# Metronlab/bow

Measured on AMD Instinct MI355X. Metric: rows/sec rolling-mean on 1B-row float64, higher is better.
Workload: dtype f64; 1 GPU; IntervalRolling(interval=10, offset=0)+Aggregate(WindowStart,ArithmeticMean), dense int64 ts=i + float64 u01 values, 1000000000 rows/GPU resident in HBM, null_count=0; rows_per_gpu=1000000000, windows_per_gpu=100000000, parallelism=rows range-partitioned x1

## Files before the change

### bow_amd/capi.py

```python
import contextlib
import ctypes as C
import os

import numpy as np

_HERE = os.path.dirname(os.path.abspath(__file__))
LIB_PATH = os.environ.get("BOWGPU_LIB") or os.path.join(_HERE, "libbowgpu.so")

FLOAT64, INT64, BOOLEAN, STRING = 1, 2, 3, 4
HOST, DEVICE, HOST_PINNED = 0, 1, 2
TYPE_NAMES = {"float64": FLOAT64, "int64": INT64, "bool": BOOLEAN, "utf8": STRING}

AGG = {
    "WindowStart": 0, "Sum": 1, "ArithmeticMean": 2, "Min": 3, "Max": 4, "Count": 5, "First": 6,
    "Last": 7, "IntegralStep": 8, "IntegralTrapezoid": 9, "WeightedAverageStep": 10,
    "WeightedAverageLinear": 11, "NumRows": 12, "Mode": 13,
}
INTERP = {"WindowStart": 0, "Linear": 1, "StepPrevious": 2, "None": 3, "Const": 4}

MAX_FACTORS = 4
BOOL_LANE_ROWS = 256
FILTER_MAX_VALUES = 32
FILTER_MAX_PREDS = 8
CARRY_MAX_AGGS = 16
# ... 148 lines not shown
    return _lib


def page_aligned(count, dtype, fill=None):
    nbytes = max(count, 1) * np.dtype(dtype).itemsize
    raw = np.empty(((nbytes + 4095) // 4096 + 1) * 4096, dtype=np.uint8)
    off = (-raw.ctypes.data) % 4096
    arr = raw[off:off + nbytes].view(dtype)
    if fill is not None:
        arr[:] = fill
    return arr


def host_register(arr):
    check(lib().bowgpu_host_register(arr.ctypes.data_as(C.c_void_p), C.c_int64(arr.nbytes)))


def host_unregister(arr):
    check(lib().bowgpu_host_unregister(arr.ctypes.data_as(C.c_void_p)))


def set_devices(ids, min_rows=None):
    ids = list(ids)
    arr = (C.c_int * max(len(ids), 1))(*ids)
    check(lib().bowgpu_set_devices(arr, len(ids)))
    if min_rows is not None:
        check(lib().bowgpu_set_fanout_min_rows(C.c_int64(min_rows)))


def get_devices():
    n = C.c_int(0)
    arr = (C.c_int * 64)()
    check(lib().bowgpu_get_devices(arr, 64, C.byref(n)))
    return [arr[i] for i in range(n.value)]


def fanout_counts():
    a, b = C.c_int64(0), C.c_int64(0)
    check(lib().bowgpu_fanout_counts(C.byref(a), C.byref(b)))
    return a.value, b.value


def last_call_ranks():
    n = C.c_int(0)
    check(lib().bowgpu_last_call_ranks(C.byref(n)))
    return n.value


class devices:

    def __init__(self, ids, min_rows=None):
        self.ids, self.min_rows = list(ids), min_rows

    def __enter__(self):
        self.prev = get_devices()
        set_devices(self.ids, self.min_rows)
        return self

    def __exit__(self, *exc):
        set_devices(self.prev, (1 << 20) if self.min_rows is not None else None)
        return False


def mem_info():
    f, t = C.c_int64(0), C.c_int64(0)
    check(lib().bowgpu_mem_info(C.byref(f), C.byref(t)))
    return f.value, t.value


def trim(all_threads=True):
    n = C.c_int64(0)
    check(lib().bowgpu_trim(1 if all_threads else 0, C.byref(n)))
    return n.value


def check(rc):
    if rc != 0:
        raise BowGpuError(rc, lib().bowgpu_last_error().decode("utf-8", "replace"))


ROUTE_NO_SIMPLE, ROUTE_FORCE_GENERAL, ROUTE_NO_LONG_ONLY, ROUTE_LONG_CLASSIC, ROUTE_LONG_STREAM_ALL = 1, 2, 4, 8, 16
ROUTE_SIMPLE_SMALL_LIST, ROUTE_SIMPLE_LARGE_LIST, ROUTE_TW_F64, ROUTE_SIMPLE_PADDED, ROUTE_INTERP_TILE = 32, 64, 128, 256, 512
ROUTE_PINNED_STAGE, ROUTE_STRICT_ORDER, ROUTE_NO_FUSED, ROUTE_TW_ROWS, ROUTE_INTERP_COPIES = 1024, 2048, 4096, 8192, 16384
ROUTE_QUEUE_HOST, ROUTE_QUEUE_DEVICE = 32768, 65536


def set_route(mask):
    check(lib().bowgpu_debug_set_route(C.c_uint32(mask)))


def get_route():
    m = C.c_uint32(0)
    check(lib().bowgpu_debug_get_route(C.byref(m)))
    return m.value


class route:

    def __init__(self, mask):
        self.mask = mask

    def __enter__(self):
        self.prev = get_route()
        set_route(self.mask)
        return self

    def __exit__(self, *exc):
        set_route(self.prev)
        return False


AGG_ROUTES = (("auto", 0), ("classic-long", ROUTE_LONG_CLASSIC), ("stream-all", ROUTE_LONG_STREAM_ALL),
              ("small-list", ROUTE_SIMPLE_SMALL_LIST), ("large-list", ROUTE_SIMPLE_LARGE_LIST), ("padded", ROUTE_SIMPLE_PADDED), ("tw-rows", ROUTE_TW_ROWS),
              ("queue-device", ROUTE_NO_LONG_ONLY | ROUTE_QUEUE_DEVICE), ("queue-host", ROUTE_NO_LONG_ONLY | ROUTE_QUEUE_HOST),
              ("lean", ROUTE_NO_SIMPLE | ROUTE_NO_LONG_ONLY), ("general", ROUTE_FORCE_GENERAL | ROUTE_NO_LONG_ONLY))
INTERP_ROUTES = (("wave3", 0), ("tile", ROUTE_INTERP_TILE))


def agg_routes():
    for label, mask in AGG_ROUTES:
        with route(mask):
            yield label


class DeviceBuffer:

    def __init__(self, nbytes):
        self.nbytes = int(nbytes)
        p = C.c_void_p()
        check(lib().bowgpu_malloc(C.byref(p), C.c_int64(self.nbytes)))
        self.ptr = p.value

    @classmethod
    def from_numpy(cls, arr):
        arr = np.ascontiguousarray(arr)
        b = cls(max(arr.nbytes, 8))
        if arr.nbytes:
            check(lib().bowgpu_memcpy_h2d(C.c_void_p(b.ptr), arr.ctypes.data_as(C.c_void_p), C.c_int64(arr.nbytes)))
        return b

    def to_numpy(self, dtype, count, first=0):
        out = np.empty(count, dtype=dtype)
        if out.nbytes:
            check(lib().bowgpu_memcpy_d2h(out.ctypes.data_as(C.c_void_p), C.c_void_p(self.ptr + first * out.itemsize), C.c_int64(out.nbytes)))
        return out

    def free(self):
        if self.ptr:
            lib().bowgpu_free(C.c_void_p(self.ptr))
            self.ptr = None

    def __del__(self):
        try:
            self.free()
        except Exception:
            pass


class Column:

    def __init__(self, values, validity=None, typ=None, offset=0, length=None, null_count=-1):
        if isinstance(values, DeviceBuffer):
            self.residency = DEVICE
            assert typ is not None and length is not None
            self.values, self.validity = values, validity
        else:
            self.residency = HOST
# ... 900 lines not shown
```

### bow_amd/csrc/agg_pass.cpp

```cpp

#include <stdio.h>
#include <stdlib.h>
#include <string.h>
#include <time.h>

#include "agg_host.h"

namespace bowgpu {

static int64_t compact_long_max_rows(uint32_t need) {
    if ((need & kNeedTimeWeighted) == kNeedTimeWeighted || (need & kNeedMinMax)) return kCompactLongBothMaxAvgRows;
    if (need & (kNeedTimeWeighted | kNeedFirstLast)) return kCompactLongMaxAvgRows;
    return 0;
}
static bool ids_and_times_fit(const Plan &plan, int64_t slot0, int64_t W) {
    const int64_t lim53 = 1ll << 53;
    return plan.first_ts > -lim53 && plan.last_ts < lim53 && (uint64_t)plan.last_ts - (uint64_t)slot0 < 0xFFFFFFF0ull && W < 0xFFFFFFF0ll;
}

int job_build(Ctx *c, const AggCall &call, const bowgpu_agg *aggs, int32_t naggs, bowgpu_out *outs, int64_t wid_base, int64_t W,
              bool holds_row0, AggJob *job, int nullable_per_pass) {
    pending_drop(c);
    const bowgpu_col *cols = call.cols;
    const int32_t ncols = call.ncols, ts_col = call.ts_col;
// ... 129 lines not shown
        const bowgpu_out *u = job->douts[i].user;
        b->user[i] = (u && u->residency == BOWGPU_DEVICE) ? u->validity : nullptr;
        b->ones[i] = all_ones || kind_never_nil(job->aggs[i].kind);
        b->count[i] = !kind_never_nil(job->aggs[i].kind);
    }
    if (preset && job->check_plan) { b->check_ts = job->P.ts; b->check_n = job->P.n; b->check_first = job->plan.first_ts; b->check_last = job->plan.last_ts; }
}

static int job_enqueue_tail(Ctx *c, AggJob *job) {
    const int64_t W = job->W;
    if (W > 0) {
        BitmapBatch b;
        job_bitmaps(job, false, false, &b);
        if (W <= kFinishHostBits) {
            BG_TRY(ctx_pinned(c, 16384, reinterpret_cast<void **>(&b.host_block)));
            job->tail_wrote_host = true;
        } else if (job->counts_used) BG_HIP(hipMemsetAsync(b.counts, 0, 8 * kMaxAggs, c->stream));
        BG_TRY(launch_finish_bitmaps(c, b));
        job->counts_used = true;
    }
    for (int i = 0; i < job->naggs; i++) BG_TRY(devout_finish(c, &job->douts[i], W, job->P.aggs[i].out_type, 0, false));
    return 0;
}

static int job_readback(Ctx *c, AggJob *job, uint32_t **hstat, uint64_t **hcnt) {
    char *hp;
    BG_TRY(ctx_pinned(c, 16384, reinterpret_cast<void **>(&hp)));
    if (job->tail_wrote_host) job->tail_wrote_host = false;
    else BG_HIP(hipMemcpyAsync(hp, job->P.status, kReadbackBytes, hipMemcpyDeviceToHost, c->stream));
    *hstat = reinterpret_cast<uint32_t *>(hp);
    *hcnt = reinterpret_cast<uint64_t *>(hp + kCountsOffset);
    return 0;
}

static int job_settle_enqueue(Ctx *c, AggJob *job, bool tail, uint32_t **hstat, uint64_t **hcnt) {
    if (tail) BG_TRY(job_enqueue_tail(c, job));
    return job_readback(c, job, hstat, hcnt);
}
static int job_settle(Ctx *c, AggJob *job, bool tail, uint32_t **hstat, uint64_t **hcnt) {
    BG_TRY(job_settle_enqueue(c, job, tail, hstat, hcnt));
    BG_HIP(hipStreamSynchronize(c->stream));
    return 0;
}

int fail_ts_unsorted() { return fail(BOWGPU_ERR_TS_UNSORTED, "interval column is not ascending: outside the device path"); }

constexpr uint32_t kLookPlan = 1u << kAggStPlanMismatch, kLookUnsorted = 1u << kAggStUnsorted, kLookOverflow = 1u << kAggStListOverflow,
                   kLookStrict = 1u << kAggStStrictTooLong;
static int agg_status_error(const uint32_t *hstat, uint32_t look) {
    if ((look & kLookPlan) && hstat[kAggStPlanMismatch])
        return fail(BOWGPU_ERR_ARG, "the plan was not made for this interval column (its first / last timestamp differ)");
    if ((look & kLookUnsorted) && hstat[kAggStUnsorted]) return fail_ts_unsorted();
    if ((look & kLookOverflow) && hstat[kAggStListOverflow]) return fail(BOWGPU_ERR_HIP, "internal: long-window list overflow");
    if ((look & kLookStrict) && hstat[kAggStStrictTooLong])
        return fail(BOWGPU_ERR_UNSUPPORTED, "strict_order: some window holds more than 2^20 rows (one lane walks a window in row order: beyond that the call is declined)");
    return 0;
}

static void job_null_counts(AggJob *job, const uint64_t *hcnt) {
    for (int i = 0; i < job->naggs; i++)
        job->douts[i].user->null_count = (job->W > 0 && !kind_never_nil(job->aggs[i].kind)) ? job->W - (int64_t)hcnt[i] : 0;
}

static bool simple_applies(const AggJob *job, bool time_weighted, bool *is_int, bool *has_nulls, bool *wide) {
    const AggParams &P = job->P;
    const Plan &plan = job->plan;
    if ((job->inclusive && !time_weighted) || !P.fits32 || job->naggs > kSimpleMaxAggs) return false;
    if (P.W <= 0) return false;

    const int64_t slot0_start = P.s0 + (int64_t)((uint64_t)P.wid_base * (uint64_t)P.interval);
    if (plan.first_ts < slot0_start && !(P.pre_rows && P.wid_base == 0)) return false;
    *wide = (uint64_t)plan.last_ts - (uint64_t)slot0_start >= 0xFFFFFFF0ull || P.W >= 0xFFFFFFF0ll;
    *is_int = true;
    *has_nulls = false;
    for (int s = 0; s < P.ncols; s++) {
        *has_nulls = *has_nulls || P.cols[s].vbits != nullptr;
        *is_int = P.cols[0].type == BOWGPU_INT64;
    }
    if ((job->need & kNeedTimeWeighted) && !time_weighted) return false;
    if (route_mask() & BOWGPU_ROUTE_NO_SIMPLE) return false;
    return true;
}

static void simple_params_build(const AggJob *job, bool wide, SimpleParams *out) {
    const AggParams &P = job->P;
    const bowgpu_agg *aggs = job->aggs;
    const int32_t naggs = job->naggs;
    SimpleParams &S = *out;
    memset(&S, 0, sizeof S);
    S.ts = P.ts;
    S.n = P.n; S.interval = P.interval; S.W = P.W;
    S.wid_base = P.wid_base;
    S.magic = P.magic;
    S.s0 = P.s0 + (int64_t)((uint64_t)P.wid_base * (uint64_t)P.interval);
    S.m32 = P.m32; S.sh1 = P.sh1_32; S.sh2 = P.sh2_32;
    S.shift_k = 0;
    if (wide) {
        int k = 0;
        while (k < 31 && !(((uint64_t)P.interval >> k) & 1ull)) k++;
        S.shift_k = k;
        interp_magic32((int64_t)((uint64_t)P.interval >> k), &S.m32, &S.sh1, &S.sh2);
    }
    S.naggs = naggs;
    S.ncols = P.ncols > 0 ? P.ncols : 1;
    S.values[0] = P.ts;
    for (int s = 0; s < P.ncols; s++) {
        S.values[s] = P.cols[s].values;
        S.vbits[s] = P.cols[s].vbits; S.vbit0[s] = P.cols[s].vbit0; S.vwords[s] = P.cols[s].vwords;
        S.col_is_int[s] = P.cols[s].type == BOWGPU_INT64;
    }
    for (int i = 0; i < naggs; i++) {
        S.kind[i] = aggs[i].kind;
        S.nfac[i] = aggs[i].n_factors;
        for (int f = 0; f < aggs[i].n_factors && f < BOWGPU_MAX_FACTORS; f++) S.fac[i][f] = aggs[i].factors[f];
        S.col[i] = P.aggs[i].slot < 0 ? 0 : P.aggs[i].slot;
        S.out_values[i] = reinterpret_cast<uint64_t *>(P.aggs[i].out_values);
        S.out_valid[i] = P.aggs[i].out_valid;
    }
    S.need = job->need;
    for (int i = 0; i < naggs; i++) {
        const int k = aggs[i].kind;
        const int cls = (k == BOWGPU_AGG_MIN || k == BOWGPU_AGG_MAX) ? 1 : (k == BOWGPU_AGG_INTEGRAL_STEP || k == BOWGPU_AGG_WAVG_STEP) ? 2
                        : (k == BOWGPU_AGG_INTEGRAL_TRAPEZOID || k == BOWGPU_AGG_WAVG_LINEAR) ? 3
                        : (k == BOWGPU_AGG_SUM || k == BOWGPU_AGG_MEAN || k == BOWGPU_AGG_FIRST || k == BOWGPU_AGG_LAST) ? 0 : 4;
        S.kind_mask[cls] |= 1u << i;
        S.col_mask[S.col[i]] |= 1u << i;
    }
    S.status = P.status; S.long_list = P.long_list; S.long_cap = P.long_cap;
    S.inclusive = job->inclusive ? 1 : 0;
    S.pre_rows = P.pre_rows;
    S.unaligned_mask = (reinterpret_cast<uintptr_t>(P.ts) & 15) ? 0x80000000u : 0u;
    for (int s = 0; s < S.ncols; s++)
        if (reinterpret_cast<uintptr_t>(S.values[s]) & 15) S.unaligned_mask |= 1u << s;
}
static int simple_launch_need(uint32_t need) { return ((need & kNeedMinMax) ? 1 : 0) | ((need & kNeedFirstLast) ? 2 : 0); }

static int job_launch_tiles(Ctx *c, AggJob *job, TileAttempt attempt, PassState *ps) {
    AggParams &P = job->P;
    const Plan &plan = job->plan;
    const int64_t W = job->W;
    const bool allow_simple = attempt != kAttemptNoSimple, force_large_list = attempt == kAttemptLargeList;
    ps->redo_with = kAttemptNone;
    if (W <= 0) { BG_HIP(hipMemsetAsync(P.status, 0, kReadbackBytes, c->stream)); return 0; }
    const uint32_t route = route_mask();
    const bool force = (route & BOWGPU_ROUTE_FORCE_GENERAL) != 0;
    const bool lean = !job->inclusive && !(job->need & kNeedTimeWeighted) && !force;
    bool is_int = false, has_nulls = false, wide = false;
    bool simple = lean && allow_simple && simple_applies(job, false, &is_int, &has_nulls, &wide);
    const bool tw = !lean && !force && allow_simple && simple_applies(job, true, &is_int, &has_nulls, &wide);
    simple = simple || tw;
    P.bits_preset = simple ? 1 : 0;
    {
        BitmapBatch b;
        job_bitmaps(job, simple, true, &b);
        BG_TRY(launch_preset_bitmaps(c, b));
        job->counts_used = false;
    }
    BG_HIP(hipEventRecord(c->ev0, c->stream));
    if (simple) {
        SimpleParams S;
        simple_params_build(job, wide, &S);
        const int64_t avg_rows = P.n / P.W;
        const bool ts32 = !P.pre_rows && ids_and_times_fit(plan, S.s0, P.W) && S.s0 > -(1ll << 53);
        const bool compact_ok = has_nulls && ts32 && !force_large_list && !(route & BOWGPU_ROUTE_TW_ROWS);
        bool compact;
        if (tw) {
            compact = compact_ok && !(route & BOWGPU_ROUTE_TW_F64) && avg_rows >= kCompactMinAvgRows;
        } else if (ps->band_rows) {
            compact = false;
        } else {
            compact = compact_ok && ((avg_rows > 128 && avg_rows <= compact_long_max_rows(job->need)) ||
                                     ((job->need & kNeedSum) && (job->need & kNeedMinMax) && avg_rows >= kCompactValuesMinAvgRows));
        }
        if (compact) {
            BG_TRY(launch_rolling_twc(c, S, avg_rows > 128));
            ps->redo_with = kAttemptLargeList;
            c->last_kernel_name = "rolling_twc_kernel";
        } else if (tw) {
            BG_TRY(launch_rolling_tw(c, S, is_int, has_nulls, wide, ts32 && !(route & BOWGPU_ROUTE_TW_F64)));
            ps->redo_with = kAttemptNoSimple;
            c->last_kernel_name = "rolling_tw_kernel";
        } else {
            const int64_t small_list_rows = rolling_simple_plain(S, is_int, has_nulls) ? 3 : 5;
            const bool dense = force_large_list || ((route & BOWGPU_ROUTE_SIMPLE_LARGE_LIST) ? true : (route & BOWGPU_ROUTE_SIMPLE_SMALL_LIST) ? false : avg_rows < small_list_rows);
            ps->redo_with = dense ? kAttemptNoSimple : kAttemptLargeList;
            BG_TRY(launch_rolling_simple(c, S, simple_launch_need(job->need), is_int, has_nulls, wide, dense));
        }
    } else if (lean && !P.pre_rows) {
        BG_TRY(launch_rolling_fast(c, P));
        c->last_kernel_name = "rolling_wave_kernel";
    } else {
        static const bool trace = [] { const char *t = getenv("BOWGPU_TRACE_ROUTE"); return t && t[0] == '1'; }();
        if (trace && !force && !(route & BOWGPU_ROUTE_NO_SIMPLE) && allow_simple)
            fprintf(stderr, "bowgpu route: general kernel (n=%lld W=%lld interval=%lld inclusive=%d naggs=%d pre_rows=%lld wid_base=%lld "
                            "fits32=%d allow_simple=%d plan=%d first_ts=%lld s0=%lld)\n", (long long)P.n, (long long)P.W,
                    (long long)P.interval, (int)job->inclusive, job->naggs, (long long)P.pre_rows, (long long)P.wid_base, (int)P.fits32,
                    (int)allow_simple, 1, (long long)plan.first_ts, (long long)P.s0);
        BG_TRY(launch_rolling_aggregate(c, P));
        c->last_kernel_name = "rolling_agg_kernel";
        c->last_slow_rows += P.n;
    }
    BG_HIP(hipEventRecord(c->ev1, c->stream));
    return 0;
}

static int long_workspace(Ctx *c, const AggParams &P, int64_t n_entries, LongWork *w) {
    const int64_t max_work = n_entries + (P.n + kLongChunkRows - 1) / kLongChunkRows;
    const int64_t scan_blocks = (n_entries + 2047) / 2048;
    auto up = [](size_t x) { return (x + 255) & ~(size_t)255; };
    const size_t b_entries = up((size_t)n_entries * long_entry_size());
    const size_t b_nchunks = up((size_t)n_entries * 4);
    const size_t b_offsets = up((size_t)(n_entries + 1) * 8);
    const size_t b_sums = up((size_t)(scan_blocks + 1) * 8);
    const size_t b_parts = up((size_t)max_work * (size_t)(P.ncols > 0 ? P.ncols : 1) * long_part_size());
    const size_t b_map = up((size_t)max_work * 4);
    void *blk;
    BG_TRY(ctx_pool(c, Ctx::kPoolSlots - 1, b_entries + b_nchunks + b_offsets + b_sums + 256 + b_map + b_parts, &blk));
    char *q = reinterpret_cast<char *>(blk);
    w->entries = q; q += b_entries;
    w->nchunks = reinterpret_cast<int32_t *>(q); q += b_nchunks;
    w->offsets = reinterpret_cast<int64_t *>(q); q += b_offsets;
    w->sums = reinterpret_cast<int64_t *>(q); q += b_sums;
    w->total = reinterpret_cast<int64_t *>(q); q += 256;
    w->work_entry = reinterpret_cast<int32_t *>(q); q += b_map;
    w->parts = q;
    w->max_work = max_work;
    return 0;
}
static int run_long_windows(Ctx *c, const AggParams &P, const uint32_t *hstat, int64_t *n_long_out, bool strict) {
    LongListStarts starts;
    starts.start[0] = 0;
    if (hstat)
        for (int s = 0; s < kLongLists; s++) starts.start[s + 1] = starts.start[s] + hstat[kLongCountWord + s];
    const int64_t n_long = hstat ? starts.start[kLongLists] : P.W;
    *n_long_out = n_long;
    if (n_long == 0) return 0;
    LongWork w;
    BG_TRY(long_workspace(c, P, n_long, &w));
    return launch_long_windows_v2(c, P, hstat ? &starts : nullptr, w.entries, w.nchunks, w.offsets, w.sums, w.total, w.work_entry, w.parts, w.max_work, strict);
}

double now_us() { timespec t; clock_gettime(CLOCK_MONOTONIC, &t); return t.tv_sec * 1e6 + t.tv_nsec * 1e-3; }

constexpr int64_t kQueueMinAvgRows = 64;
static int job_queue_enqueue(Ctx *c, AggJob *job, PassState *ps) {
    if (!ps->queue) return 0;
    const AggParams &P = job->P;
    BG_TRY(launch_long_queue(c, P, P.long_cap * kLongLists, ps->qw.entries, ps->qw.nchunks, job->strict ? ((int64_t)1 << 20) : kQueueWalkMaxRows, job->strict));
    BG_HIP(hipEventRecord(c->ev1, c->stream));
    return 0;
}

static int job_report_ms(Ctx *c, bool ran, double *kernel_ms) {
    float ms = 0;
    if (ran) BG_HIP(hipEventElapsedTime(&ms, c->ev0, c->ev1));
    c->last_kernel_ms = ms;
    if (kernel_ms) *kernel_ms = ms;
    return 0;
}

int job_pass_enqueue(Ctx *c, AggJob *job, bool finish, PassState *ps) {
    {
        const uint32_t route = route_mask();
        const int64_t avg_rows = job->W > 0 ? job->P.n / job->W : 0;
        ps->queue = job->W > 0 && !(route & BOWGPU_ROUTE_QUEUE_HOST) && (avg_rows >= kQueueMinAvgRows || (route & BOWGPU_ROUTE_QUEUE_DEVICE));
        if (ps->queue) BG_TRY(long_workspace(c, job->P, job->P.long_cap * kLongLists, &ps->qw));
    }
    BG_TRY(job_launch_tiles(c, job, kAttemptFirst, ps));
// ... 183 lines not shown
```

### bow_amd/csrc/common.h

```cpp
#pragma once

#include <hip/hip_runtime.h>
#include <stdint.h>

#include <string>
#include <vector>

#include "../../include/bowgpu.h"
#include "bit_span.h"
#include "debug_routes.h"

namespace bowgpu {

void set_error(const char *fmt, ...);
int fail(int code, const char *fmt, ...);
int fail_ts_unsorted();
int hip_fail(hipError_t e, const char *what);

#define BG_HIP(expr)                                         \
    do {                                                     \
        hipError_t _e = (expr);                              \
        if (_e != hipSuccess) return hip_fail(_e, #expr);    \
    } while (0)

// ... 282 lines not shown
    const void *values[kMaxCols];
    const uint32_t *vbits[kMaxCols];
    int64_t vbit0[kMaxCols], vwords[kMaxCols];
    int32_t col_is_int[kMaxCols];
    int32_t kind[kSimpleMaxAggs];
    int32_t col[kSimpleMaxAggs];
    int32_t nfac[kSimpleMaxAggs];
    double fac[kSimpleMaxAggs][BOWGPU_MAX_FACTORS];
    uint64_t *out_values[kSimpleMaxAggs];
    uint32_t *out_valid[kSimpleMaxAggs];
    uint32_t *status;
    int64_t *long_list;
    int64_t long_cap;
};
int launch_rolling_simple(Ctx *c, const SimpleParams &p, int need, bool is_int, bool has_nulls, bool wide, bool dense);
bool rolling_simple_plain(const SimpleParams &p, bool is_int, bool has_nulls);
int launch_rolling_tw(Ctx *c, const SimpleParams &p, bool is_int, bool has_nulls, bool wide, bool ts32);

struct FusedCol {
    int32_t type, kind;
    int32_t has_prev, prev_t_valid, prev_v_valid, next_valid;
    double const_value, prev_t, prev_v, next_t, next_v;
    int64_t prev_v_i64;
};
struct FusedParams {
    SimpleParams s;
    FusedCol cols[kMaxCols];
    double inv_interval;
};
int launch_rolling_fused(Ctx *c, const FusedParams &fp, int need, bool has_nulls);
int interp_validate(const bowgpu_col *cols, int32_t ncols, int32_t ts_col, const bowgpu_options *o, const bowgpu_interp *interps, int32_t ninterps);

int launch_rolling_twc(Ctx *c, const SimpleParams &p, bool long_halo = false);
constexpr int64_t kCompactLongMaxAvgRows = 255;
constexpr int64_t kCompactLongBothMaxAvgRows = 176;
constexpr int64_t kCompactValuesMinAvgRows = 48;
constexpr int64_t kCompactMinAvgRows = 12;
int launch_rolling_aggregate(Ctx *c, const AggParams &p);
int launch_rolling_fast(Ctx *c, const AggParams &p);
constexpr int kLongChunkRows = 4096;
constexpr int kLongStreamRows = 512;
constexpr int64_t kLongOnlyAvgRows = 128;
constexpr int64_t kLongStreamAnyAvgRows = 129;
constexpr int64_t kLongBisectAvgRows = 512;
constexpr int64_t kLongClassicAvgRows = 1ll << 22;
constexpr int kLongLists = 64;
constexpr int kLongCountWord = 16;
constexpr int kStatusWords = kLongCountWord + kLongLists;
constexpr int kAggStUnsorted = 0;
constexpr int kAggStListOverflow = 2;
constexpr int kAggStRedo = 4;
constexpr int kAggStFusedDeclines = 5;
constexpr int kAggStPlanMismatch = 6;
constexpr int kAggStStrictTooLong = 7;
struct LongListStarts { int64_t start[kLongLists + 1]; };
size_t long_entry_size();
size_t long_part_size();
int stream_rw_run(Ctx *c, const void *a, const void *b, int64_t bytes_each, void *o0, void *o1, int64_t rows_per_slot, int64_t nslots, bool nt,
                  int reps, float *ms);
int stream_sum_run(Ctx *c, const void *a, const void *b, int64_t bytes_each, int mode, int blocks_per_cu, int reps, uint64_t *d_out, float *ms);
int launch_long_windows_v2(Ctx *c, const AggParams &p, const LongListStarts *starts, void *entries, int32_t *nchunks, int64_t *offsets,
                           int64_t *block_sums, int64_t *d_total, int32_t *work_entry, void *partials, int64_t max_work, bool strict = false,
                           int64_t n_given = 0);
int launch_long_queue(Ctx *c, const AggParams &p, int64_t capacity, void *big_entries, int32_t *big_nchunks, int64_t walk_max_rows, bool strict);
constexpr int kQueueBigWord = 8;
constexpr int64_t kQueueWalkMaxRows = 1024;
size_t long_stream_workspace(int64_t n, int64_t W, int ncols);
int launch_long_stream(Ctx *c, const AggParams &p, void *workspace);
int launch_fix_tail_bits(Ctx *c, uint8_t *bitmap, int64_t nbits);
struct BitmapBatch {
    int32_t n, status_words;
    int64_t nbits;
    uint32_t *work[kMaxAggs];
    uint8_t *user[kMaxAggs];
    int32_t ones[kMaxAggs];
    int32_t count[kMaxAggs];
    uint32_t *status;
    unsigned long long *counts;
    char *host_block;
    const int64_t *check_ts;
    int64_t check_n, check_first, check_last;
};
constexpr int64_t kFinishHostBits = 262144;
int launch_preset_bitmaps(Ctx *c, const BitmapBatch &b);
int launch_finish_bitmaps(Ctx *c, const BitmapBatch &b);
int launch_popcount(Ctx *c, const uint32_t *words, int64_t bit0, int64_t nbits, uint64_t *d_count);
int launch_fetch_two(Ctx *c, const int64_t *col, int64_t i0, int64_t i1, int64_t *host_out);

int launch_mode(Ctx *c, const int64_t *ts, const int64_t *first_idx, int64_t n, int64_t s0, int64_t interval, int64_t W, int pre_rows,
                int inclusive, const void *values,
                const uint32_t *vbits, int64_t vbit0, int is_int, const bowgpu_agg *agg, void *out_values, uint32_t *out_valid,
                int64_t *n_mid, int64_t *n_long);

constexpr int kBoolMaxOuts = 16;
constexpr int kBoolLaneRows = 256;
struct BoolOut {
    int32_t kind, nfac;
    double fac[BOWGPU_MAX_FACTORS];
    void *values;
    uint32_t *valid;
};
struct BoolParams {
    const int64_t *ts, *first_idx;
    int64_t s0, n, interval, W;
    int32_t pre_rows, inclusive;
    const uint32_t *tbits, *vbits;
    int64_t tbit0, vbit0;
    unsigned long long *null_windows;
    int32_t nouts, _pad;
    BoolOut outs[kBoolMaxOuts];
};
int launch_bool_windows(Ctx *c, const BoolParams &P);
int launch_bool_widen(Ctx *c, const uint32_t *tbits, int64_t tbit0, const uint32_t *vbits, int64_t vbit0, int64_t n, double *out, uint32_t *out_valid);

struct NbrIndex {
    const int64_t *prev_before;
    const int64_t *next_after;
    int64_t g0;
};
int launch_ts_nullfill(Ctx *c, const int64_t *ts, const uint32_t *tbits, int64_t tbit0, int64_t n, const struct NbrIndex &ix, int64_t s0, int64_t interval,
                       const MagicDiv &magic, int inclusive, int64_t *ts_eff, uint64_t *keep, uint64_t *plain, unsigned long long *d_dropped);
struct QuirkFixAgg {
    const void *values; const uint32_t *vbits; int64_t vbit0;
    uint64_t *out_values; uint32_t *out_valid;
    int32_t type, kind, n_factors, _pad;
    double factors[BOWGPU_MAX_FACTORS];
};
struct QuirkFix { int32_t naggs, _pad; QuirkFixAgg a[8]; };
int launch_ts_quirk_fix(Ctx *c, const int64_t *ts, const uint32_t *tbits, int64_t tbit0, int64_t n, const struct NbrIndex &ix, int64_t s0, int64_t interval,
                        const MagicDiv &magic, int64_t W, const QuirkFix &fx, unsigned long long *d_fixed);
int launch_count_to_f64(Ctx *c, uint64_t *v, const uint32_t *valid, int64_t n, int n_factors, const double *factors);
int fetch_valid(Ctx *c, const bowgpu_col *col, int64_t row, int *valid);
constexpr int kMaxCompactCols = 16;
struct CompactCols {
    int32_t ncols, ts_col;
    const uint64_t *values[kMaxCompactCols]; const uint32_t *vbits[kMaxCompactCols]; int64_t vbit0[kMaxCompactCols];
    uint64_t *out_values[kMaxCompactCols];
    uint64_t *lookup_bits[kMaxCompactCols];
    uint64_t *patch_values[kMaxCompactCols]; uint32_t *patch_valid[kMaxCompactCols];
    uint64_t *ts_bits;
};
struct PatchInterps {
    int64_t m;
    const uint64_t *both_bits[kMaxCompactCols];
    NbrIndex nbr[kMaxCompactCols];
    int32_t type[kMaxCompactCols], kind[kMaxCompactCols], has_prev[kMaxCompactCols], prev_t_valid[kMaxCompactCols], prev_v_valid[kMaxCompactCols];
    double const_value[kMaxCompactCols], prev_t[kMaxCompactCols], prev_v[kMaxCompactCols];
    int64_t prev_v_i64[kMaxCompactCols];
};
int launch_keep_counts(Ctx *c, const uint64_t *keep, int64_t nw, int32_t *counts);
int launch_compact_rows(Ctx *c, const uint64_t *keep, const int64_t *base, int64_t n, const int64_t *ts_eff, const uint32_t *tbits, int64_t tbit0,
                        const uint64_t *plain, const CompactCols &cc, int64_t *marker, uint32_t *flags);
int launch_pack_flags(Ctx *c, const uint32_t *flags, int64_t m, const CompactCols &cc, uint64_t *marker_bits);
int launch_interp_patch(Ctx *c, const int64_t *marker_out, const uint32_t *marker_valid, int64_t m_out, const uint32_t *flags, const CompactCols &cc,
                        const PatchInterps &px);
int launch_and_bits(Ctx *c, const uint32_t *a, int64_t abit0, const uint32_t *b, int64_t bbit0, int64_t n, uint64_t *out);

int launch_range_state(Ctx *c, const AggParams &p, int mode, uint64_t wid, const bowgpu_carry_state *d_seeds,
                       bowgpu_carry_state *d_states_out, const bowgpu_next_row *d_next, int seed_alive, int strict);

int launch_fill_empty(Ctx *c, const AggParams &p, int64_t slot0, int64_t slot1);

int launch_window_first_rows(Ctx *c, const int64_t *ts, int64_t n, const Plan &plan, int64_t *first_idx, uint32_t *status);
int launch_exclusive_scan(Ctx *c, const int32_t *in, int64_t n, int64_t *out, int64_t *block_sums, int64_t *d_total);
int launch_col_order(Ctx *c, const uint64_t *values, const uint32_t *vbits, int64_t vbit0, int64_t n, int32_t type, uint32_t *d_flags);
int launch_window_bounds(Ctx *c, const int64_t *ts, int64_t n, const Plan &plan, int inclusive, int pre_rows,
// ... 362 lines not shown
```

### bow_amd/csrc/debug_routes.h

```cpp
#pragma once
enum {
    BOWGPU_ROUTE_NO_SIMPLE = 1,
    BOWGPU_ROUTE_FORCE_GENERAL = 2,
    BOWGPU_ROUTE_NO_LONG_ONLY = 4,
    BOWGPU_ROUTE_LONG_CLASSIC = 8,
    BOWGPU_ROUTE_LONG_STREAM_ALL = 16,
    BOWGPU_ROUTE_SIMPLE_SMALL_LIST = 32,
    BOWGPU_ROUTE_SIMPLE_LARGE_LIST = 64,
    BOWGPU_ROUTE_TW_F64 = 128,
    BOWGPU_ROUTE_SIMPLE_PADDED = 256,
    BOWGPU_ROUTE_INTERP_TILE = 512,
    BOWGPU_ROUTE_NO_FUSED = 4096,
    BOWGPU_ROUTE_TW_ROWS = 8192,
    BOWGPU_ROUTE_INTERP_COPIES = 16384,
    BOWGPU_ROUTE_QUEUE_HOST = 32768,
    BOWGPU_ROUTE_QUEUE_DEVICE = 65536,
    BOWGPU_ROUTE__ALL = 131071
};
```

### bow_amd/csrc/rolling_agg.hip

```cpp

#include "agg_device.h"

namespace bowgpu {

namespace {

constexpr int kBlock = 256;
constexpr int kTile = 2048;
constexpr int kHalo = 128;
constexpr int kRows = kTile + kHalo;
constexpr int kChunks = kTile / (2 * kBlock);
constexpr int kCnt = kChunks * 4 + 1;
constexpr int kSpanBits = 2048 + 64;
constexpr int kSpanWords = kSpanBits / 32;
constexpr int kMaxNullable = 8;
constexpr int kGapInline = 4;
constexpr int kGapList = 64;

struct TileShared {
    uint64_t val[kRows];
    uint32_t seg_wid[kRows + 2];
    uint16_t seg_row[kRows + 2];
    uint32_t vbits[kRows / 32 + 2];
    uint32_t obits[kMaxNullable][kSpanWords];
// ... 376 lines not shown
    if (a == 0 && blockIdx.x == 0) {
        for (int i = threadIdx.x; i < b.status_words; i += blockDim.x)
            b.status[i] = (i == kAggStPlanMismatch && b.check_ts && b.check_n > 0 && (b.check_ts[0] != b.check_first || b.check_ts[b.check_n - 1] != b.check_last)) ? 1u : 0u;
        if (threadIdx.x < kMaxAggs) b.counts[threadIdx.x] = 0ull;
    }
    if (a >= b.n) return;
    const int64_t nwords = (b.nbits + 31) >> 5;
    const uint32_t fill = b.ones[a] ? 0xFFFFFFFFu : 0u;
    uint32_t *w = b.work[a];
    for (int64_t i = (int64_t)blockIdx.x * blockDim.x + threadIdx.x; i < nwords; i += (int64_t)gridDim.x * blockDim.x) {
        uint32_t x = fill;
        if (i == nwords - 1 && (b.nbits & 31)) x &= (1u << (b.nbits & 31)) - 1u;
        w[i] = x;
    }
}
__global__ __launch_bounds__(256) void finish_bitmaps_kernel(const BitmapBatch b) {
    const int a = blockIdx.y;
    if (a >= b.n) return;
    const int64_t nwords = (b.nbits + 31) >> 5, nbytes = (b.nbits + 7) >> 3;
    const uint32_t *w = b.work[a];
    uint8_t *u = b.user[a];
    const bool aligned = (reinterpret_cast<uintptr_t>(u) & 3) == 0;
    unsigned long long acc = 0;
    const bool vec = (reinterpret_cast<uintptr_t>(w) & 15) == 0 && (!u || (reinterpret_cast<uintptr_t>(u) & 15) == 0);
    const int64_t nvec = vec ? ((b.nbits >> 5) >> 2) : 0;
    const int64_t stride = (int64_t)gridDim.x * blockDim.x;
    int64_t g = (int64_t)blockIdx.x * blockDim.x + threadIdx.x;
    for (; g + 3 * stride < nvec; g += 4 * stride) {
        const uint4 *q = reinterpret_cast<const uint4 *>(w) + g;
        const uint4 x0 = q[0], x1 = q[stride], x2 = q[2 * stride], x3 = q[3 * stride];
        if (b.count[a]) acc += __popc(x0.x) + __popc(x0.y) + __popc(x0.z) + __popc(x0.w) + __popc(x1.x) + __popc(x1.y) + __popc(x1.z) + __popc(x1.w) +
                               __popc(x2.x) + __popc(x2.y) + __popc(x2.z) + __popc(x2.w) + __popc(x3.x) + __popc(x3.y) + __popc(x3.z) + __popc(x3.w);
        if (u) {
            uint4 *d = reinterpret_cast<uint4 *>(u) + g;
            d[0] = x0; d[stride] = x1; d[2 * stride] = x2; d[3 * stride] = x3;
        }
    }
    for (; g < nvec; g += stride) {
        const uint4 x = reinterpret_cast<const uint4 *>(w)[g];
        if (b.count[a]) acc += __popc(x.x) + __popc(x.y) + __popc(x.z) + __popc(x.w);
        if (u) reinterpret_cast<uint4 *>(u)[g] = x;
    }
    for (int64_t i = 4 * nvec + (int64_t)blockIdx.x * blockDim.x + threadIdx.x; i < nwords; i += (int64_t)gridDim.x * blockDim.x) {
        uint32_t x = w[i];
        if (i == nwords - 1 && (b.nbits & 31)) x &= (1u << (b.nbits & 31)) - 1u;
        if (b.count[a]) acc += __popc(x);
        if (u) {
            if (aligned && 4 * i + 4 <= nbytes) reinterpret_cast<uint32_t *>(u)[i] = x;
            else for (int k = 0; k < 4 && 4 * i + k < nbytes; k++) u[4 * i + k] = (uint8_t)(x >> (8 * k));
        }
    }
    if (b.count[a]) {
        __shared__ unsigned long long wave_sum[4];
        for (int o = 32; o > 0; o >>= 1) acc += __shfl_down(acc, o);
        if ((threadIdx.x & 63) == 0) wave_sum[threadIdx.x >> 6] = acc;
        __syncthreads();
        if (threadIdx.x == 0) {
            const unsigned long long t = wave_sum[0] + wave_sum[1] + wave_sum[2] + wave_sum[3];
            if (b.host_block) reinterpret_cast<unsigned long long *>(b.host_block + 1024)[a] = t;
            else if (t) atomicAdd(&b.counts[a], t);
        }
    } else if (b.host_block && threadIdx.x == 0) reinterpret_cast<unsigned long long *>(b.host_block + 1024)[a] = 0;
    if (b.host_block && a == 0 && blockIdx.x == 0)
        for (int t = threadIdx.x; t < b.status_words; t += blockDim.x) reinterpret_cast<uint32_t *>(b.host_block)[t] = b.status[t];
}

static unsigned bitmap_grid(int64_t nbits) {
    const int64_t nwords = (nbits + 31) >> 5;
    int64_t g = (nwords + 255) / 256;
    return (unsigned)(g < 1 ? 1 : g > 1024 ? 1024 : g);
}
int launch_preset_bitmaps(Ctx *c, const BitmapBatch &b) {
    hipLaunchKernelGGL(preset_bitmaps_kernel, dim3(bitmap_grid(b.nbits), b.n > 0 ? b.n : 1), dim3(256), 0, c->stream, b);
    BG_HIP(hipGetLastError());
    return 0;
}
int launch_finish_bitmaps(Ctx *c, const BitmapBatch &b) {
    if (b.n <= 0 || b.nbits <= 0) return 0;
    hipLaunchKernelGGL(finish_bitmaps_kernel, dim3(b.host_block ? 1u : bitmap_grid(b.nbits), b.n), dim3(256), 0, c->stream, b);
    BG_HIP(hipGetLastError());
    return 0;
}

int launch_fix_tail_bits(Ctx *c, uint8_t *bitmap, int64_t nbits) {
    if ((nbits & 7) == 0) return 0;
    hipLaunchKernelGGL(fix_tail_bits_kernel, dim3(1), dim3(64), 0, c->stream, bitmap, nbits);
    BG_HIP(hipGetLastError());
    return 0;
}

__global__ void fetch_two_kernel(const int64_t *col, int64_t i0, int64_t i1, int64_t *host_out) {
    if (threadIdx.x == 0) host_out[0] = col[i0];
    if (threadIdx.x == 1) host_out[1] = col[i1];
}
int launch_fetch_two(Ctx *c, const int64_t *col, int64_t i0, int64_t i1, int64_t *host_out) {
    hipLaunchKernelGGL(fetch_two_kernel, dim3(1), dim3(64), 0, c->stream, col, i0, i1, host_out);
    BG_HIP(hipGetLastError());
    return 0;
}

int launch_popcount(Ctx *c, const uint32_t *words, int64_t bit0, int64_t nbits, uint64_t *d_count) {
    BG_HIP(hipMemsetAsync(d_count, 0, 8, c->stream));
    if (nbits <= 0) return 0;
    const int64_t nwords = (nbits + 63) / 32;
    int64_t grid = (nwords + 255) / 256;
    if (grid > 512) grid = 512;
    hipLaunchKernelGGL(popcount_kernel, dim3((unsigned)grid), dim3(256), 0, c->stream, words, bit0, nbits,
                       reinterpret_cast<unsigned long long *>(d_count));
    BG_HIP(hipGetLastError());
    return 0;
}

}
```

Baseline: 319.6 billion rows/s.

## Split WindowStart output into a separate streaming fill kernel

WindowStart aggregates are taken out of the simple rolling tile kernel and written by a dedicated kernel that computes s0+k*interval per window and stores 16-byte pairs with nontemporal stores. The tile kernel then handles only the remaining aggregates, which lowers its per-window output work and register use. The cost is one extra kernel launch and a separate output pass over W windows. A debug route keeps the old in-tile behaviour available.

```diff
diff --git a/bow_amd/capi.py b/bow_amd/capi.py
--- a/bow_amd/capi.py
+++ b/bow_amd/capi.py
@@ -254,7 +254,7 @@
 ROUTE_NO_SIMPLE, ROUTE_FORCE_GENERAL, ROUTE_NO_LONG_ONLY, ROUTE_LONG_CLASSIC, ROUTE_LONG_STREAM_ALL = 1, 2, 4, 8, 16
 ROUTE_SIMPLE_SMALL_LIST, ROUTE_SIMPLE_LARGE_LIST, ROUTE_TW_F64, ROUTE_SIMPLE_PADDED, ROUTE_INTERP_TILE = 32, 64, 128, 256, 512
 ROUTE_PINNED_STAGE, ROUTE_STRICT_ORDER, ROUTE_NO_FUSED, ROUTE_TW_ROWS, ROUTE_INTERP_COPIES = 1024, 2048, 4096, 8192, 16384
-ROUTE_QUEUE_HOST, ROUTE_QUEUE_DEVICE = 32768, 65536
+ROUTE_QUEUE_HOST, ROUTE_QUEUE_DEVICE, ROUTE_WS_IN_TILE = 32768, 65536, 131072
 
 
 def set_route(mask):
diff --git a/bow_amd/csrc/agg_pass.cpp b/bow_amd/csrc/agg_pass.cpp
--- a/bow_amd/csrc/agg_pass.cpp
+++ b/bow_amd/csrc/agg_pass.cpp
@@ -235,12 +235,12 @@
     return true;
 }
 
-static void simple_params_build(const AggJob *job, bool wide, SimpleParams *out) {
+static void simple_params_build(const AggJob *job, bool wide, SimpleParams *out, WsFill *fill = nullptr) {
     const AggParams &P = job->P;
     const bowgpu_agg *aggs = job->aggs;
-    const int32_t naggs = job->naggs;
     SimpleParams &S = *out;
     memset(&S, 0, sizeof S);
+    if (fill) memset(fill, 0, sizeof *fill);
     S.ts = P.ts;
     S.n = P.n; S.interval = P.interval; S.W = P.W;
     S.wid_base = P.wid_base;
@@ -254,7 +254,6 @@
         S.shift_k = k;
         interp_magic32((int64_t)((uint64_t)P.interval >> k), &S.m32, &S.sh1, &S.sh2);
     }
-    S.naggs = naggs;
     S.ncols = P.ncols > 0 ? P.ncols : 1;
     S.values[0] = P.ts;
     for (int s = 0; s < P.ncols; s++) {
@@ -262,23 +261,33 @@
         S.vbits[s] = P.cols[s].vbits; S.vbit0[s] = P.cols[s].vbit0; S.vwords[s] = P.cols[s].vwords;
         S.col_is_int[s] = P.cols[s].type == BOWGPU_INT64;
     }
-    for (int i = 0; i < naggs; i++) {
-        S.kind[i] = aggs[i].kind;
-        S.nfac[i] = aggs[i].n_factors;
-        for (int f = 0; f < aggs[i].n_factors && f < BOWGPU_MAX_FACTORS; f++) S.fac[i][f] = aggs[i].factors[f];
-        S.col[i] = P.aggs[i].slot < 0 ? 0 : P.aggs[i].slot;
-        S.out_values[i] = reinterpret_cast<uint64_t *>(P.aggs[i].out_values);
-        S.out_valid[i] = P.aggs[i].out_valid;
-    }
     S.need = job->need;
-    for (int i = 0; i < naggs; i++) {
+    int32_t m = 0;
+    for (int i = 0; i < job->naggs; i++) {
         const int k = aggs[i].kind;
+        const int nfac = aggs[i].n_factors < BOWGPU_MAX_FACTORS ? aggs[i].n_factors : BOWGPU_MAX_FACTORS;
+        if (fill && k == BOWGPU_AGG_WINDOW_START) {
+            const int w = fill->n++;
+            fill->nfac[w] = nfac;
+            for (int f = 0; f < nfac; f++) fill->fac[w][f] = aggs[i].factors[f];
+            fill->out[w] = reinterpret_cast<uint64_t *>(P.aggs[i].out_values);
+            continue;
+        }
+        S.kind[m] = k;
+        S.nfac[m] = aggs[i].n_factors;
+        for (int f = 0; f < nfac; f++) S.fac[m][f] = aggs[i].factors[f];
+        S.col[m] = P.aggs[i].slot < 0 ? 0 : P.aggs[i].slot;
+        S.out_values[m] = reinterpret_cast<uint64_t *>(P.aggs[i].out_values);
+        S.out_valid[m] = P.aggs[i].out_valid;
         const int cls = (k == BOWGPU_AGG_MIN || k == BOWGPU_AGG_MAX) ? 1 : (k == BOWGPU_AGG_INTEGRAL_STEP || k == BOWGPU_AGG_WAVG_STEP) ? 2
                         : (k == BOWGPU_AGG_INTEGRAL_TRAPEZOID || k == BOWGPU_AGG_WAVG_LINEAR) ? 3
                         : (k == BOWGPU_AGG_SUM || k == BOWGPU_AGG_MEAN || k == BOWGPU_AGG_FIRST || k == BOWGPU_AGG_LAST) ? 0 : 4;
-        S.kind_mask[cls] |= 1u << i;
-        S.col_mask[S.col[i]] |= 1u << i;
-    }
+        S.kind_mask[cls] |= 1u << m;
+        S.col_mask[S.col[m]] |= 1u << m;
+        m++;
+    }
+    S.naggs = m;
+    if (fill) { fill->W = S.W; fill->s0 = S.s0; fill->interval = S.interval; }
     S.status = P.status; S.long_list = P.long_list; S.long_cap = P.long_cap;
     S.inclusive = job->inclusive ? 1 : 0;
     S.pre_rows = P.pre_rows;
@@ -337,6 +346,11 @@
             const int64_t small_list_rows = rolling_simple_plain(S, is_int, has_nulls) ? 3 : 5;
             const bool dense = force_large_list || ((route & BOWGPU_ROUTE_SIMPLE_LARGE_LIST) ? true : (route & BOWGPU_ROUTE_SIMPLE_SMALL_LIST) ? false : avg_rows < small_list_rows);
             ps->redo_with = dense ? kAttemptNoSimple : kAttemptLargeList;
+            if (!(route & BOWGPU_ROUTE_WS_IN_TILE)) {
+                WsFill fill;
+                simple_params_build(job, wide, &S, &fill);
+                BG_TRY(launch_ws_fill(c, fill));
+            }
             BG_TRY(launch_rolling_simple(c, S, simple_launch_need(job->need), is_int, has_nulls, wide, dense));
         }
     } else if (lean && !P.pre_rows) {
diff --git a/bow_amd/csrc/common.h b/bow_amd/csrc/common.h
--- a/bow_amd/csrc/common.h
+++ b/bow_amd/csrc/common.h
@@ -388,6 +388,14 @@
     int64_t check_n, check_first, check_last;
 };
 constexpr int64_t kFinishHostBits = 262144;
+struct WsFill {
+    int32_t n;
+    int32_t nfac[kSimpleMaxAggs];
+    int64_t W, s0, interval;
+    uint64_t *out[kSimpleMaxAggs];
+    double fac[kSimpleMaxAggs][BOWGPU_MAX_FACTORS];
+};
+int launch_ws_fill(Ctx *c, const WsFill &f);
 int launch_preset_bitmaps(Ctx *c, const BitmapBatch &b);
 int launch_finish_bitmaps(Ctx *c, const BitmapBatch &b);
 int launch_popcount(Ctx *c, const uint32_t *words, int64_t bit0, int64_t nbits, uint64_t *d_count);
diff --git a/bow_amd/csrc/debug_routes.h b/bow_amd/csrc/debug_routes.h
--- a/bow_amd/csrc/debug_routes.h
+++ b/bow_amd/csrc/debug_routes.h
@@ -15,5 +15,6 @@
     BOWGPU_ROUTE_INTERP_COPIES = 16384,
     BOWGPU_ROUTE_QUEUE_HOST = 32768,
     BOWGPU_ROUTE_QUEUE_DEVICE = 65536,
-    BOWGPU_ROUTE__ALL = 131071
+    BOWGPU_ROUTE_WS_IN_TILE = 131072,
+    BOWGPU_ROUTE__ALL = 262143
 };
diff --git a/bow_amd/csrc/rolling_agg.hip b/bow_amd/csrc/rolling_agg.hip
--- a/bow_amd/csrc/rolling_agg.hip
+++ b/bow_amd/csrc/rolling_agg.hip
@@ -482,6 +482,41 @@
     return 0;
 }
 
+typedef unsigned long long ws_pair __attribute__((ext_vector_type(2)));
+__global__ __launch_bounds__(256) void ws_fill_kernel(const WsFill f) {
+    const int a = blockIdx.y;
+    uint64_t *__restrict__ out = f.out[a];
+    const int nf = f.nfac[a];
+    const uint64_t s0 = (uint64_t)f.s0, iv = (uint64_t)f.interval;
+    auto value = [&](int64_t k) -> uint64_t {
+        const uint64_t bits = s0 + (uint64_t)k * iv;
+        return nf ? apply_factors(bits, true, nf, f.fac[a]) : bits;
+    };
+    const int64_t head = (reinterpret_cast<uintptr_t>(out) & 15) ? 1 : 0;
+    const int64_t npairs = (f.W - head) >> 1;
+    const int64_t tail = head + 2 * npairs;
+    if (blockIdx.x == 0 && threadIdx.x == 0) {
+        if (head) out[0] = value(0);
+        if (tail < f.W) out[tail] = value(tail);
+    }
+    ws_pair *__restrict__ out2 = reinterpret_cast<ws_pair *>(out + head);
+    for (int64_t j = (int64_t)blockIdx.x * blockDim.x + threadIdx.x; j < npairs; j += (int64_t)gridDim.x * blockDim.x) {
+        const int64_t k = head + 2 * j;
+        ws_pair v;
+        v.x = value(k);
+        v.y = value(k + 1);
+        __builtin_nontemporal_store(v, &out2[j]);
+    }
+}
+int launch_ws_fill(Ctx *c, const WsFill &f) {
+    if (f.n <= 0 || f.W <= 0) return 0;
+    int64_t g = ((f.W + 1) / 2 + 255) / 256;
+    if (g > 0x7FFFFFFFll) g = 0x7FFFFFFFll;
+    hipLaunchKernelGGL(ws_fill_kernel, dim3((unsigned)g, (unsigned)f.n), dim3(256), 0, c->stream, f);
+    BG_HIP(hipGetLastError());
+    return 0;
+}
+
 int launch_fix_tail_bits(Ctx *c, uint8_t *bitmap, int64_t nbits) {
     if ((nbits & 7) == 0) return 0;
     hipLaunchKernelGGL(fix_tail_bits_kernel, dim3(1), dim3(64), 0, c->stream, bitmap, nbits);
```

After: 332.5 billion rows/s, median of 6. +4.1%, better.
